# lzhangbj/deep_video_interpolation_extrapolation

Hardware: AMD Instinct MI355X
Metric: train frames/s (256x512 len-3 clips) (higher is better)
Workload: dtype bf16; 1 GPU; InterNet int_5_len_3 train step 256x512 bf16; per_gpu_batch=8, global_batch=8, parallelism=dp1, step=eager, executor side-stream lanes

## Files before the change

deep_video_interpolation_extrapolation_amd/_lib.py:

```python
import ctypes
import os
import threading

import torch

LIB_PATH = os.path.join(os.path.dirname(os.path.abspath(__file__)), "libdvie.so")

DVIE_OK = 0
DVIE_EINVAL = 1001
F32, BF16 = 0, 1
ACT_NONE, ACT_LRELU, ACT_ELU, ACT_RELU, ACT_TANH = 0, 1, 2, 3, 4
EW_FUSE, EW_UPT, EW_POOL, EW_POOLT, EW_COPY, EW_L1SIGN, EW_NCHW, EW_TONCHW, EW_MASK, EW_IM2COL, EW_LABELS = range(11)
LOSS_L1, LOSS_GDL, LOSS_SSIM, LOSS_MSE, LOSS_CE, LOSS_L1NHWC, LOSS_COSNHWC, LOSS_IOU, LOSS_ARGMAX_IOU = range(9)
OP_CONV, OP_WGRAD, OP_WREDUCE, OP_COLSUM, OP_EW, OP_LOSS, OP_PACK = 1, 2, 3, 4, 5, 6, 7
OP_BN_FWD, OP_BN_BWD, OP_HEAD_FWD, OP_HEAD_BWD, OP_ATTN, OP_HEAD3_BWD, OP_SEGENC_FWD = 8, 9, 10, 11, 12, 13, 14
OP_SEGENC_BWD = 15
OP_WREDUCE_MULTI = 16
OP_COSFEAT = 17
COSFEAT_MAX_TAPS = 8
YUV_420, YUV_444 = 420, 444
(ATTN_L2NORM, ATTN_L2NORM_BWD, ATTN_CORR, ATTN_GATHER, ATTN_GATHER_T, ATTN_SOFTMAX, ATTN_SOFTMAX_BWD, ATTN_WNORM,
 ATTN_WNORM_BWD, ATTN_POOL, ATTN_POOL_T) = range(11)

vp = ctypes.c_void_p
# ... 214 lines not shown

class AttnDesc(ctypes.Structure):
    _fields_ = [
        ("a", vp), ("b0", vp), ("b1", vp), ("y", vp), ("res", vp), ("z", vp),
        ("a_ld", i64), ("b_ld", i64), ("y_ld", i64), ("res_ld", i64), ("z_ld", i64),
        ("op", i32), ("n", i32), ("h", i32), ("w", i32),
        ("c", i32), ("wh", i32), ("ww", i32), ("nhalf", i32),
        ("half0", i32), ("act", i32), ("dact", i32), ("beta", i32),
        ("dtype", i32), ("pad0", i32),
        ("alpha", f32), ("pad1", f32),
    ]


class PackList(ctypes.Structure):
    _fields_ = [("descs_dev", vp), ("n", i32), ("blocks", i32)]


class Head3BwdDesc(ctypes.Structure):
    _fields_ = [
        ("g", vp), ("h", vp), ("wd", vp), ("dh", vp), ("ws", vp),
        ("g_ld", i64), ("h_ld", i64), ("dh_ld", i64),
        ("n", i32), ("hgt", i32), ("wid", i32), ("c", i32),
        ("cout", i32), ("kpad", i32), ("dy0", i32), ("dx0", i32),
        ("splits", i32), ("dact", i32),
        ("alpha", f32), ("pad0", f32),
    ]


class SegencDesc(ctypes.Structure):
    _fields_ = [
        ("inp", vp), ("e1", vp), ("e2", vp), ("out", vp), ("w0", vp), ("w2", vp), ("w4", vp),
        ("b0", vp), ("b2", vp), ("b4", vp),
        ("in_ld", i64), ("e1_ld", i64), ("e2_ld", i64), ("out_ld", i64),
        ("n", i32), ("h", i32), ("w", i32), ("kpad0", i32), ("kpad2", i32), ("kpad4", i32),
    ]


class SegencBwdDesc(ctypes.Structure):
    _fields_ = [
        ("dout", vp), ("e2", vp), ("e1", vp), ("inp", vp), ("w4d", vp), ("w2d", vp),
        ("dw4", vp), ("dw2", vp), ("dw0", vp), ("db4", vp), ("db2", vp), ("db0", vp),
        ("dout_ld", i64), ("e2_ld", i64), ("e1_ld", i64), ("in_ld", i64),
        ("n", i32), ("h", i32), ("w", i32), ("kpad4", i32), ("kpad2", i32), ("slabs", i32),
    ]


class WreduceMultiDesc(ctypes.Structure):
    _fields_ = [("descs", vp), ("n", i32), ("pad", i32)]


class _OpUnion(ctypes.Union):
    _fields_ = [
        ("conv", ConvDesc), ("wgrad", WgradDesc), ("wreduce", WreduceDesc), ("colsum", ColsumDesc),
        ("ew", EwDesc), ("loss", LossDesc), ("pack", PackList), ("bn", BnDesc), ("head", HeadDesc),
        ("attn", AttnDesc), ("head3", Head3BwdDesc), ("segenc", SegencDesc), ("segenc_bwd", SegencBwdDesc),
        ("wreduce_multi", WreduceMultiDesc), ("cosfeat", CosFeatDesc),
    ]


class Op(ctypes.Structure):
    _fields_ = [("kind", i32), ("lane", i32), ("u", _OpUnion)]


_ABI = {0: Op, OP_CONV: ConvDesc, OP_WGRAD: WgradDesc, OP_WREDUCE: WreduceDesc, OP_COLSUM: ColsumDesc,
        OP_EW: EwDesc, OP_LOSS: LossDesc, OP_PACK: PackDesc, OP_BN_FWD: BnDesc, OP_HEAD_FWD: HeadDesc,
        OP_ATTN: AttnDesc, OP_HEAD3_BWD: Head3BwdDesc, OP_SEGENC_FWD: SegencDesc, OP_SEGENC_BWD: SegencBwdDesc, OP_WREDUCE_MULTI: WreduceMultiDesc,
        OP_COSFEAT: CosFeatDesc, 100: WarpDesc, 101: SoftmaxDesc, 102: SnLayer, 103: ClipDesc,
        104: SynthLoadDesc, 105: SynthFinishDesc, 106: SynthBridgeDesc, 107: SynthScoreDesc,
        108: SynthLoadPadDesc, 109: SynthFinishCropDesc, 110: SynthVggLoadDesc}
_ABI_MORE = {111: SynthMsssimDesc, 112: SynthYuvDesc}

EXPORTS = [
    "dvie_conv2d_fwd", "dvie_conv2d_wgrad", "dvie_wgrad_splits_hint", "dvie_wgrad_slabs", "dvie_wgrad_reduce", "dvie_wgrad_reduce_multi", "dvie_colsum", "dvie_pack_weights",
    "dvie_ew", "dvie_loss", "dvie_loss_partial_count", "dvie_loss_ws_floats", "dvie_warp_fwd",
    "dvie_warp_bwd", "dvie_adamax", "dvie_scale", "dvie_run_ops", "dvie_abi_sizeof", "dvie_version",
    "dvie_last_error", "dvie_bn_fwd", "dvie_bn_bwd", "dvie_bn_partial_splits", "dvie_head_fwd", "dvie_head_bwd",
    "dvie_softmax_fwd", "dvie_softmax_bwd", "dvie_adam", "dvie_sn_fwd", "dvie_sn_bwd", "dvie_reparam_fwd",
    "dvie_reparam_bwd", "dvie_warp_ws_floats", "dvie_clip_prep", "dvie_attn", "dvie_step_inc", "dvie_adamax_dev",
    "dvie_adam_dev", "dvie_mfma_probe", "dvie_launch_probe", "dvie_sum_f32", "dvie_wgrad_bias_slabs", "dvie_head3_bwd",
    "dvie_segenc_fwd", "dvie_segenc_bwd", "dvie_pack_blocks", "dvie_trace_kernels", "dvie_traced_kernels",
    "dvie_synth_load", "dvie_synth_finish", "dvie_synth_bridge", "dvie_synth_score", "dvie_synth_score_ws_bytes",
    "dvie_synth_load_pad", "dvie_synth_finish_crop", "dvie_conv_zbits", "dvie_bn_partial_doubles",
    "dvie_synth_vgg_load", "dvie_cosfeat", "dvie_cosfeat_blocks", "dvie_synth_msssim", "dvie_synth_msssim_ws_bytes",
    "dvie_synth_yuv2rgb", "dvie_synth_rgb2yuv",
]

_lib = None
_lock = threading.Lock()


class DvieError(RuntimeError):
    pass


def load():
    global _lib
    if _lib is not None:
        return _lib
    with _lock:
        if _lib is not None:
            return _lib
        if not os.path.exists(LIB_PATH):
            raise DvieError(
                f"{LIB_PATH} is missing: build it with `python -c 'import __graft_entry__ as g; g.build()'` "
                "(there is no non-HIP fallback)")
        lib = ctypes.CDLL(LIB_PATH)
        lib.dvie_abi_sizeof.restype = ctypes.c_size_t
        lib.dvie_abi_sizeof.argtypes = [i32]
        for which, st in {**_ABI, **_ABI_MORE}.items():
            got = lib.dvie_abi_sizeof(which)
            if got != ctypes.sizeof(st):
                raise DvieError(f"ABI mismatch for {st.__name__}: C {got} vs ctypes {ctypes.sizeof(st)}")
        lib.dvie_version.restype = ctypes.c_char_p
        lib.dvie_last_error.restype = ctypes.c_char_p
        for name in ("dvie_conv2d_fwd", "dvie_conv2d_wgrad", "dvie_wgrad_reduce", "dvie_colsum", "dvie_ew",
                     "dvie_loss", "dvie_warp_fwd", "dvie_warp_bwd", "dvie_bn_fwd", "dvie_bn_bwd", "dvie_head_fwd",
                     "dvie_head_bwd", "dvie_softmax_fwd", "dvie_softmax_bwd", "dvie_clip_prep", "dvie_attn",
                     "dvie_head3_bwd", "dvie_segenc_fwd", "dvie_segenc_bwd", "dvie_synth_load", "dvie_synth_finish",
                     "dvie_synth_bridge", "dvie_synth_score", "dvie_synth_load_pad", "dvie_synth_finish_crop",
                     "dvie_synth_vgg_load", "dvie_cosfeat", "dvie_synth_msssim", "dvie_synth_yuv2rgb",
                     "dvie_synth_rgb2yuv"):
            getattr(lib, name).argtypes = [vp, vp]
            getattr(lib, name).restype = i32
        lib.dvie_pack_weights.argtypes = [vp, i32, i32, vp]
        lib.dvie_wgrad_reduce_multi.argtypes = [vp, i32, vp]
        lib.dvie_wgrad_reduce_multi.restype = i32
        lib.dvie_trace_kernels.argtypes = [i32]
        lib.dvie_trace_kernels.restype = i32
        lib.dvie_traced_kernels.argtypes = []
        lib.dvie_traced_kernels.restype = ctypes.c_char_p
        for name in ("dvie_wgrad_splits_hint", "dvie_wgrad_slabs", "dvie_bn_partial_splits", "dvie_pack_blocks",
                     "dvie_conv_zbits", "dvie_cosfeat_blocks"):
            getattr(lib, name).argtypes = [vp]
            getattr(lib, name).restype = i32
        lib.dvie_run_ops.argtypes = [vp, i32, vp]
        lib.dvie_loss_partial_count.argtypes = [vp]
        lib.dvie_loss_partial_count.restype = ctypes.c_size_t
        lib.dvie_warp_ws_floats.argtypes = [vp]
        lib.dvie_warp_ws_floats.restype = ctypes.c_size_t
        lib.dvie_loss_ws_floats.argtypes = [vp]
        lib.dvie_loss_ws_floats.restype = ctypes.c_size_t
        lib.dvie_bn_partial_doubles.argtypes = [vp]
        lib.dvie_bn_partial_doubles.restype = ctypes.c_size_t
        lib.dvie_synth_score_ws_bytes.argtypes = [vp]
        lib.dvie_synth_score_ws_bytes.restype = ctypes.c_size_t
        lib.dvie_synth_msssim_ws_bytes.argtypes = [vp]
        lib.dvie_synth_msssim_ws_bytes.restype = ctypes.c_size_t
        lib.dvie_adamax.argtypes = [vp, vp, vp, vp, i64, f32, f32, f32, f32, f32, vp]
        lib.dvie_scale.argtypes = [vp, i64, f32, vp]
        lib.dvie_adam.argtypes = [vp, vp, vp, vp, i64, f32, f32, f32, f32, f32, vp]
        f64 = ctypes.c_double
        lib.dvie_adamax_dev.argtypes = [vp, vp, vp, vp, i64, f64, f64, f64, f64, f64, vp, vp]
        lib.dvie_adam_dev.argtypes = [vp, vp, vp, vp, i64, f64, f64, f64, f64, f64, vp, vp]
        lib.dvie_step_inc.argtypes = [vp, vp]
        lib.dvie_mfma_probe.argtypes = [vp, i32, i32, vp]
        lib.dvie_mfma_probe.restype = i32
        lib.dvie_launch_probe.argtypes = [i32, i32, vp]
        lib.dvie_launch_probe.restype = i32
        lib.dvie_sum_f32.argtypes = [vp, i32, vp, vp]
        lib.dvie_sum_f32.restype = i32
        lib.dvie_wgrad_bias_slabs.argtypes = [vp]
        lib.dvie_wgrad_bias_slabs.restype = i32
        for name in ("dvie_sn_fwd", "dvie_sn_bwd"):
            getattr(lib, name).argtypes = [vp, i32, vp, vp]
            getattr(lib, name).restype = i32
        lib.dvie_reparam_fwd.argtypes = [vp, vp, vp, vp, i64, vp]
        lib.dvie_reparam_bwd.argtypes = [vp, vp, vp, vp, vp, i64, i32, vp]
        lib.dvie_reparam_fwd.restype = lib.dvie_reparam_bwd.restype = i32
        _lib = lib
        return lib


def check(rc, what=""):
    if rc != DVIE_OK:
        msg = load().dvie_last_error().decode(errors="replace") if rc == DVIE_EINVAL else f"hipError {rc}"
        raise DvieError(f"{what}: {msg}")


def stream_ptr(device=None):
    return torch.cuda.current_stream(device).cuda_stream


def require_gpu(t):
    if not t.is_cuda:
        raise DvieError("dvie ops run on the MI355X only: tensor is on %s (no CPU fallback)" % t.device)
```

deep_video_interpolation_extrapolation_amd/csrc/conv1x1.hip:

```cpp
#include <stdlib.h>

#include "conv_epilogue.h"

namespace dvie {

typedef __attribute__((address_space(3))) void* lds_ptr_1x1;

#define DVIE_VMCNT1(N) __builtin_amdgcn_s_waitcnt(((N) & 15) | (((N) >> 4) << 14) | (7 << 4) | (15 << 8))

__device__ __forceinline__ void transpose8x8(i32x4 (&ob)[8], int lane) {
  const int b = lane & 7;
#pragma unroll
  for (int d = 4; d >= 1; d >>= 1) {
    const bool up = (b & d) != 0;
#pragma unroll
    for (int k = 0; k < 8; ++k) {
      if (k & d) continue;
      i32x4 t, r;
#pragma unroll
      for (int e = 0; e < 4; ++e) t[e] = up ? ob[k][e] : ob[k + d][e];
#pragma unroll
      for (int e = 0; e < 4; ++e) r[e] = __shfl_xor(t[e], d);
#pragma unroll
      for (int e = 0; e < 4; ++e) {
// ... 750 lines not shown
      if (p.act == DVIE_ACT_LRELU) switch (dbg_env() & 7) {
#define DVIE_RING_AB(V)                                                                                                \
  case V:                                                                                                              \
    DVIE_LAUNCH((conv1x1_ring_kernel<TMC, NWP, MI, NWC, DVIE_ACT_LRELU, V>), dim3(256), dim3(64 * NW), 0, s, p, n_ct, \
                n_tiles);                                                                                              \
    return;
          DVIE_RING_AB(1) DVIE_RING_AB(2) DVIE_RING_AB(3) DVIE_RING_AB(4) DVIE_RING_AB(5) DVIE_RING_AB(6) DVIE_RING_AB(7)
#undef DVIE_RING_AB
          default: break;
        }
#endif
      if (p.act == DVIE_ACT_LRELU && p.zbits)
        DVIE_LAUNCH((conv1x1_ring_kernel<TMC, NWP, MI, NWC, DVIE_ACT_LRELU, 0, true>), dim3(256), dim3(64 * NW), 0, s, p, n_ct, n_tiles);
      else if (p.act == DVIE_ACT_LRELU)
        DVIE_LAUNCH((conv1x1_ring_kernel<TMC, NWP, MI, NWC, DVIE_ACT_LRELU>), dim3(256), dim3(64 * NW), 0, s, p, n_ct, n_tiles);
      else
        DVIE_LAUNCH((conv1x1_ring_kernel<TMC, NWP, MI, NWC, DVIE_ACT_NONE>), dim3(256), dim3(64 * NW), 0, s, p, n_ct, n_tiles);
      return;
    }
  }
  if constexpr (NS >= 2 && NS <= 5 && MI * TMC <= 4) {
    const int per_cu = 163840 / C::SMEM;
    const int G = 256 * (per_cu > 2 ? 2 : per_cu);
    if (p.c > KC && n_tiles > G) {
      DVIE_LAUNCH((conv1x1_persist_kernel<TMC, NS, KC, NWP, MI, NWC>), dim3(G), dim3(64 * NW), 0, s, p, n_ct,
                         n_tiles);
      return;
    }
  }
  const bool ident = ident_out(p);
  int pre = 0;
  if constexpr (NS == 1) {
    if (ident && p.c <= KC) {
      pre = MI * TMC > 4 ? 0 : (p.res ? 1 : 0) | (p.beta ? 2 : 0) | (p.dact ? 4 : 0);
      if ((pre & 4) && zb_reads(p)) pre |= 8;
      if (p.zbits && p.act) pre |= 16;
    }
  }
  if constexpr (NS == 1 && MI == 1 && 2 * TMC == 8) {
    if (ident && ce_env_on() && p.cout % C::BC == 0) {
      switch (pre) {
#define DVIE_CE_CASE(V)                                                                                              \
  case V:                                                                                                            \
    DVIE_LAUNCH((conv1x1_kernel<TMC, NS, KC, NWP, MI, NWC, false, PreOk<V, NS, MI * TMC, TMC>::v, true>), dim3(n_tiles), \
                       dim3(64 * NW), 0, s, p, n_ct, n_tiles, 0);                                                     \
    return;
        DVIE_CE_CASE(0) DVIE_CE_CASE(1) DVIE_CE_CASE(2) DVIE_CE_CASE(3) DVIE_CE_CASE(4)
        DVIE_CE_CASE(5) DVIE_CE_CASE(6) DVIE_CE_CASE(7)
        DVIE_CE_CASE(12) DVIE_CE_CASE(13) DVIE_CE_CASE(14) DVIE_CE_CASE(15) DVIE_CE_CASE(16) DVIE_CE_CASE(17)
#undef DVIE_CE_CASE
      }
    }
  }
  switch (pre) {
#define DVIE_PRE_CASE(V)                                                                                          \
  case V:                                                                                                        \
    DVIE_LAUNCH((conv1x1_kernel<TMC, NS, KC, NWP, MI, NWC, false, PreOk<V, NS, MI * TMC, TMC>::v>), dim3(n_tiles), \
                       dim3(64 * NW), 0, s, p, n_ct, n_tiles, dbg_env());                                                   \
    break;
    DVIE_PRE_CASE(1) DVIE_PRE_CASE(2) DVIE_PRE_CASE(3) DVIE_PRE_CASE(4) DVIE_PRE_CASE(5)
    DVIE_PRE_CASE(6) DVIE_PRE_CASE(7)
    DVIE_PRE_CASE(12) DVIE_PRE_CASE(13) DVIE_PRE_CASE(14) DVIE_PRE_CASE(15) DVIE_PRE_CASE(16) DVIE_PRE_CASE(17)
#undef DVIE_PRE_CASE
    default:
      DVIE_LAUNCH((conv1x1_kernel<TMC, NS, KC, NWP, MI, NWC, false>), dim3(n_tiles), dim3(64 * NW), 0, s, p, n_ct, n_tiles, dbg_env());
  }
}

static bool takes_1x1(const dvie_conv_desc& p) {
  if (p.dtype != DVIE_BF16 || p.th != 1 || p.tw != 1) return false;
  if (p.sy != 1 || p.sx != 1 || p.dy0 != 0 || p.dx0 != 0 || p.ih != p.oh || p.iw != p.ow) return false;
  if (p.osy < 1 || p.osx < 1 || p.ory < 0 || p.orx < 0) return false;
  if (p.c % 64 != 0 && p.c > 64) return false;
  if ((long long)p.n * p.oh * p.ow >= (1LL << 31)) return false;
  return true;
}

int conv1x1_zbits(const dvie_conv_desc& p) {
  if (!takes_1x1(p)) return -1;
  if (zb_writes(p)) return tile_1x1(p) == T_WIDE ? 2 : 1;
  return zb_reads(p);
}

bool conv1x1_launch(const dvie_conv_desc& p, hipStream_t s) {
  if (!takes_1x1(p)) return false;
  switch (tile_1x1(p)) {
    case T_2_1: launch_1x1<2, 1>(p, s); break;
    case T_2_3: launch_1x1<2, 3>(p, s); break;
    case T_4_3: launch_1x1<4, 3>(p, s); break;
    case T_4_1: launch_1x1<4, 1>(p, s); break;
    case T_WIDE: launch_1x1<4, 2, 64, 4, 2, 2>(p, s); break;
  }
  return true;
}

}
```

deep_video_interpolation_extrapolation_amd/csrc/warp_optim.hip:

```cpp
#include <stdlib.h>

#include <algorithm>

#include "common.h"

namespace dvie {

__device__ __forceinline__ float linspace_pm1(int i, int n) {
  if (n <= 1) return -1.f;
  const float step = 2.f / (float)(n - 1);
  return (i < n / 2) ? __builtin_fmaf(step, (float)i, -1.f) : __builtin_fmaf(-step, (float)(n - 1 - i), 1.f);
}

__device__ __forceinline__ float unnorm(float g, int size, int ac) {
  return ac ? ((g + 1.f) / 2.f) * (float)(size - 1) : ((g + 1.f) * (float)size - 1.f) / 2.f;
}

struct WarpTap {
  int x0, y0;
  float ix, iy, wnw, wne, wsw, wse;
  bool vx0, vx1, vy0, vy1;
};

__device__ __forceinline__ WarpTap warp_tap(int x, int y, float fx, float fy, int w, int h, int ac) {
  WarpTap t;
  const float gx = linspace_pm1(x, w) - fx;
  const float gy = linspace_pm1(y, h) - fy;
  t.ix = unnorm(gx, w, ac);
  t.iy = unnorm(gy, h, ac);
  t.x0 = (int)floorf(t.ix);
  t.y0 = (int)floorf(t.iy);
  const int x1 = t.x0 + 1, y1 = t.y0 + 1;
  t.wnw = ((float)x1 - t.ix) * ((float)y1 - t.iy);
  t.wne = (t.ix - (float)t.x0) * ((float)y1 - t.iy);
  t.wsw = ((float)x1 - t.ix) * (t.iy - (float)t.y0);
  t.wse = (t.ix - (float)t.x0) * (t.iy - (float)t.y0);
  t.vx0 = t.x0 >= 0 && t.x0 < w;
  t.vx1 = x1 >= 0 && x1 < w;
  t.vy0 = t.y0 >= 0 && t.y0 < h;
  t.vy1 = y1 >= 0 && y1 < h;
  return t;
}

__device__ __forceinline__ __amdgpu_buffer_rsrc_t warp_plane(const float* im, long long hw) {
  return __builtin_amdgcn_make_buffer_rsrc((void*)im, 0, (int)(hw * 4), 0x00020000);
}

__device__ __forceinline__ void warp_corners(__amdgpu_buffer_rsrc_t im, const WarpTap& t, int w, float& a, float& b,
                                             float& c, float& d, bool pair = false) {
  constexpr unsigned kOut = 0x80000000u;
  const unsigned r0 = (unsigned)(t.y0 * w), r1 = (unsigned)((t.y0 + 1) * w);
  if (pair) {
    const auto u = __builtin_amdgcn_raw_buffer_load_b64(im, t.vy0 ? (r0 + t.x0) * 4u : kOut, 0, 0);
    const auto v = __builtin_amdgcn_raw_buffer_load_b64(im, t.vy1 ? (r1 + t.x0) * 4u : kOut, 0, 0);
    a = __uint_as_float(u[0]);
    b = __uint_as_float(u[1]);
    c = __uint_as_float(v[0]);
    d = __uint_as_float(v[1]);
    return;
  }
  const unsigned oa = (t.vy0 && t.vx0) ? (r0 + t.x0) * 4u : kOut;
  const unsigned ob = (t.vy0 && t.vx1) ? (r0 + t.x0 + 1) * 4u : kOut;
  const unsigned oc = (t.vy1 && t.vx0) ? (r1 + t.x0) * 4u : kOut;
  const unsigned od = (t.vy1 && t.vx1) ? (r1 + t.x0 + 1) * 4u : kOut;
  a = __builtin_bit_cast(float, __builtin_amdgcn_raw_buffer_load_b32(im, oa, 0, 0));
  b = __builtin_bit_cast(float, __builtin_amdgcn_raw_buffer_load_b32(im, ob, 0, 0));
  c = __builtin_bit_cast(float, __builtin_amdgcn_raw_buffer_load_b32(im, oc, 0, 0));
  d = __builtin_bit_cast(float, __builtin_amdgcn_raw_buffer_load_b32(im, od, 0, 0));
}

__device__ __forceinline__ float warp_blend(float a, float b, float c, float d, const WarpTap& t) {
  float v = 0.f;
  v += a * t.wnw;
  v += b * t.wne;
  v += c * t.wsw;
  v += d * t.wse;
  return v;
}

template <int CC, int LAUX = 0, int SAUX = 0, int WPB = 4>
__global__ __launch_bounds__(64 * WPB) void warp_fwd_kernel(const dvie_warp_desc p, int xcd) {
  const int segs = (p.w + 255) >> 8;
  const long long hw = (long long)p.h * p.w;
  const int waves = p.n * p.h * segs;
  const int lane = threadIdx.x & 63;
// ... 415 lines not shown
  if (n == 0) return DVIE_OK;
  DVIE_LAUNCH(adamax_kernel, dim3(grid_for(n)), dim3(256), 0, (hipStream_t)stream, p, g, m, u, n, clr, b1, b2,
                     eps, wd, (const float*)nullptr, 0.0, 0.0);
  DVIE_RETURN_LAUNCH();
}

int dvie_adamax_dev(float* p, const float* g, float* m, float* u, long long n, double lr, double b1, double b2,
                    double eps, double wd, const float* step, void* stream) {
  DVIE_CHECK_ARG(p && g && m && u && step && n >= 0, "adamax_dev: args");
  if (n == 0) return DVIE_OK;
  DVIE_LAUNCH(adamax_kernel, dim3(grid_for(n)), dim3(256), 0, (hipStream_t)stream, p, g, m, u, n, 0.f,
                     (float)b1, (float)b2, (float)eps, (float)wd, step, lr, b1);
  DVIE_RETURN_LAUNCH();
}

int dvie_step_inc(float* step, void* stream) {
  DVIE_CHECK_ARG(step, "step_inc: null");
  DVIE_LAUNCH(step_inc_kernel, dim3(1), dim3(64), 0, (hipStream_t)stream, step);
  DVIE_RETURN_LAUNCH();
}

int dvie_scale(float* p, long long n, float s, void* stream) {
  DVIE_CHECK_ARG(p && n >= 0, "scale: args");
  if (n == 0) return DVIE_OK;
  DVIE_LAUNCH(scale_kernel, dim3(grid_for(n)), dim3(256), 0, (hipStream_t)stream, p, n, s);
  DVIE_RETURN_LAUNCH();
}

}

namespace {
struct DevLanes {
  hipStream_t side = nullptr;
  hipEvent_t join = nullptr, tail = nullptr;
  bool ok = false;
};
thread_local DevLanes dev_lanes[64];

DevLanes* lanes_of_device() {
  int dev = 0;
  if (hipGetDevice(&dev) != hipSuccess || dev < 0 || dev >= 64) return nullptr;
  DevLanes& d = dev_lanes[dev];
  if (!d.ok) {
    int least = 0, greatest = 0;
    if (hipDeviceGetStreamPriorityRange(&least, &greatest) != hipSuccess) least = 0;
    if (hipStreamCreateWithPriority(&d.side, hipStreamNonBlocking, least) != hipSuccess ||
        hipEventCreateWithFlags(&d.join, hipEventDisableTiming) != hipSuccess ||
        hipEventCreateWithFlags(&d.tail, hipEventDisableTiming) != hipSuccess)
      return nullptr;
    d.ok = true;
  }
  return &d;
}

bool lanes_on() {
  const char* e = getenv("DVIE_OP_LANES");
  return !(e && *e == '0');
}

struct LaneRun {
  DevLanes* d = nullptr;
  hipStream_t main = nullptr;
  bool tail_fresh = false;
  bool used = false;

  hipError_t enter_weight() {
    hipError_t e = hipSuccess;
    if (!tail_fresh) {
      e = hipEventRecord(d->tail, main);
      if (e == hipSuccess) e = hipStreamWaitEvent(d->side, d->tail, 0);
      tail_fresh = true;
    }
    used = true;
    return e;
  }
  hipError_t finish() {
    if (!used) return hipSuccess;
    hipError_t e = hipEventRecord(d->join, d->side);
    return e == hipSuccess ? hipStreamWaitEvent(main, d->join, 0) : e;
  }
};
}

extern "C" {

int dvie_run_ops(const dvie_op* ops, int n, void* stream) {
  LaneRun lr;
  lr.main = (hipStream_t)stream;
  hipStreamCaptureStatus cap = hipStreamCaptureStatusNone;
  const bool capturing = hipStreamIsCapturing(lr.main, &cap) == hipSuccess && cap != hipStreamCaptureStatusNone;
  const bool lanes = lanes_on() && !capturing;
  auto finish = [&](int rc) {
    if (lr.d) {
      const hipError_t e = lr.finish();
      if (rc == DVIE_OK && e != hipSuccess) {
        set_error("run_ops: lane join failed");
        return (int)e;
      }
    }
    return rc;
  };
  for (int i = 0; i < n; ++i) {
    int rc = DVIE_OK;
    const dvie_op& o = ops[i];
    if (o.lane < 0 || o.lane > 1) {
      set_error("run_ops: lane %d of op %d out of range", o.lane, i);
      return finish(DVIE_EINVAL);
    }
    hipStream_t st = lr.main;
    if (lanes && o.lane == 1) {
      if (!lr.d) lr.d = lanes_of_device();
      if (!lr.d) {
        set_error("run_ops: side stream unavailable");
        return finish(DVIE_EINVAL);
      }
      if (lr.enter_weight() != hipSuccess) {
        set_error("run_ops: weight-lane wait failed at op %d", i);
        return finish(DVIE_EINVAL);
      }
      st = lr.d->side;
    } else {
      lr.tail_fresh = false;
    }
    void* s = (void*)st;
#ifdef DVIE_TIMING_DBG
    static const long long skip_kinds = getenv("DVIE_SKIP_KINDS") ? atoll(getenv("DVIE_SKIP_KINDS")) : 0;
    if ((skip_kinds >> o.kind) & 1) continue;
#endif
    switch (o.kind) {
      case DVIE_OP_CONV: rc = dvie_conv2d_fwd(&o.u.conv, s); break;
      case DVIE_OP_WGRAD: rc = dvie_conv2d_wgrad(&o.u.wgrad, s); break;
      case DVIE_OP_WREDUCE: rc = dvie_wgrad_reduce(&o.u.wreduce, s); break;
      case DVIE_OP_WREDUCE_MULTI: rc = dvie_wgrad_reduce_multi(o.u.wreduce_multi.descs, o.u.wreduce_multi.n, s); break;
      case DVIE_OP_COLSUM: rc = dvie_colsum(&o.u.colsum, s); break;
      case DVIE_OP_EW: rc = dvie_ew(&o.u.ew, s); break;
      case DVIE_OP_LOSS: rc = dvie_loss(&o.u.loss, s); break;
      case DVIE_OP_PACK: rc = dvie_pack_weights(o.u.pack.descs_dev, o.u.pack.n, o.u.pack.blocks, s); break;
      case DVIE_OP_BN_FWD: rc = dvie_bn_fwd(&o.u.bn, s); break;
      case DVIE_OP_BN_BWD: rc = dvie_bn_bwd(&o.u.bn, s); break;
      case DVIE_OP_HEAD_FWD: rc = dvie_head_fwd(&o.u.head, s); break;
      case DVIE_OP_HEAD_BWD: rc = dvie_head_bwd(&o.u.head, s); break;
      case DVIE_OP_ATTN: rc = dvie_attn(&o.u.attn, s); break;
      case DVIE_OP_HEAD3_BWD: rc = dvie_head3_bwd(&o.u.head3, s); break;
      case DVIE_OP_SEGENC_FWD: rc = dvie_segenc_fwd(&o.u.segenc, s); break;
      case DVIE_OP_SEGENC_BWD: rc = dvie_segenc_bwd(&o.u.segenc_bwd, s); break;
      case DVIE_OP_COSFEAT: rc = dvie_cosfeat(&o.u.cosfeat, s); break;
      default: set_error("run_ops: unknown op kind %d at %d", o.kind, i); return finish(DVIE_EINVAL);
    }
    if (rc != DVIE_OK) {
      if (rc == DVIE_EINVAL) {
        char buf[512];
        snprintf(buf, sizeof(buf), "op %d (kind %d): %s", i, o.kind, dvie_last_error());
        set_error("%s", buf);
      }
      return finish(rc);
    }
  }
  return finish(DVIE_OK);
}

size_t dvie_abi_sizeof(int which) {
  switch (which) {
    case 0: return sizeof(dvie_op);
    case DVIE_OP_CONV: return sizeof(dvie_conv_desc);
    case DVIE_OP_WGRAD: return sizeof(dvie_wgrad_desc);
    case DVIE_OP_WREDUCE: return sizeof(dvie_wreduce_desc);
    case DVIE_OP_WREDUCE_MULTI: return sizeof(dvie_wreduce_multi_desc);
    case DVIE_OP_COLSUM: return sizeof(dvie_colsum_desc);
    case DVIE_OP_EW: return sizeof(dvie_ew_desc);
    case DVIE_OP_LOSS: return sizeof(dvie_loss_desc);
    case DVIE_OP_PACK: return sizeof(dvie_pack_desc);
    case DVIE_OP_BN_FWD: return sizeof(dvie_bn_desc);
    case DVIE_OP_HEAD_FWD: return sizeof(dvie_head_desc);
    case DVIE_OP_ATTN: return sizeof(dvie_attn_desc);
    case DVIE_OP_HEAD3_BWD: return sizeof(dvie_head3_bwd_desc);
    case DVIE_OP_SEGENC_FWD: return sizeof(dvie_segenc_desc);
    case DVIE_OP_SEGENC_BWD: return sizeof(dvie_segenc_bwd_desc);
    case DVIE_OP_COSFEAT: return sizeof(dvie_cosfeat_desc);
    case 100: return sizeof(dvie_warp_desc);
    case 101: return sizeof(dvie_softmax_desc);
    case 102: return sizeof(dvie_sn_layer);
    case 103: return sizeof(dvie_clip_desc);
    case 104: return sizeof(dvie_synth_load_desc);
    case 105: return sizeof(dvie_synth_finish_desc);
    case 106: return sizeof(dvie_synth_bridge_desc);
    case 107: return sizeof(dvie_synth_score_desc);
    case 108: return sizeof(dvie_synth_load_pad_desc);
    case 109: return sizeof(dvie_synth_finish_crop_desc);
    case 110: return sizeof(dvie_synth_vgg_load_desc);
    case 111: return sizeof(dvie_synth_msssim_desc);
    case 112: return sizeof(dvie_synth_yuv_desc);
    default: return 0;
  }
}

const char* dvie_version(void) { return "dvie 0.1.0 gfx950"; }

}
```

include/dvie.h:

```cpp
#ifndef DVIE_H
#define DVIE_H

#include <stddef.h>
#include <stdint.h>

#ifdef __cplusplus
extern "C" {
#endif

#define DVIE_OK 0
#define DVIE_EINVAL 1001

#define DVIE_F32 0
#define DVIE_BF16 1

#define DVIE_ACT_NONE 0
#define DVIE_ACT_LRELU 1
#define DVIE_ACT_ELU 2
#define DVIE_ACT_RELU 3
#define DVIE_ACT_TANH 4

typedef struct dvie_conv_desc {
  const void* x;
  const void* w;
  void* y;
  const float* bias;
  const void* res;
  const void* z;
  long long x_ld, y_ld, res_ld, z_ld;
  int n, ih, iw, c;
  int kpad, cout;
  int oh, ow, sy, sx;
  int th, tw, dy0, dx0, ddy, ddx;
  int yh, yw, osy, osx, ory, orx;
  int act, dact, beta, dtype;
  int out_f32;
  float alpha;
  int phc;
  int pad1;
  void* zbits;
  long long zbits_ld;
} dvie_conv_desc;

int dvie_conv2d_fwd(const dvie_conv_desc* d, void* stream);

int dvie_conv_zbits(const dvie_conv_desc* d);

typedef struct dvie_wgrad_desc {
  const void* g;
  const void* x;
  float* ws;
  long long g_ld, x_ld;
  int n, oh, ow, cout;
  int ih, iw, c, sy;
  int sx, th, tw, dy0;
  int dx0, ddy, ddx, splits;
  int dtype;
  int tmap;
  float* bws;
  int ws_taps;
  int pad1;
} dvie_wgrad_desc;

int dvie_conv2d_wgrad(const dvie_wgrad_desc* d, void* stream);

int dvie_wgrad_bias_slabs(const dvie_wgrad_desc* d);

int dvie_wgrad_splits_hint(const dvie_wgrad_desc* d);

int dvie_wgrad_slabs(const dvie_wgrad_desc* d);

typedef struct dvie_wreduce_desc {
  const float* ws;
  float* dw;
  const int* cmap;
  int splits, ws_rows, ws_k, co_off;
  int cout_p, cin_p, kh_n, kw_n;
  int c, beta;
} dvie_wreduce_desc;

int dvie_wgrad_reduce(const dvie_wreduce_desc* d, void* stream);

int dvie_wgrad_reduce_multi(const dvie_wreduce_desc* descs, int n, void* stream);
typedef struct dvie_wreduce_multi_desc {
  const dvie_wreduce_desc* descs;
  int n, pad;
} dvie_wreduce_multi_desc;

typedef struct dvie_colsum_desc {
  const void* g;
  float* ws;
  long long g_ld;
  long long rows;
  int c, splits, dtype, pad0;
} dvie_colsum_desc;

int dvie_colsum(const dvie_colsum_desc* d, void* stream);

typedef struct dvie_pack_desc {
  const float* src;
  void* dst;
  const int* cmap;
  int rows, kpad, c, mode;
  int th, tw, kh0, kw0;
  int dkh, dkw, cout_s, cin_s;
  int kh_s, kw_s, dtype, blk0;
} dvie_pack_desc;

int dvie_pack_weights(const dvie_pack_desc* descs_dev, int n, int blocks, void* stream);

int dvie_pack_blocks(const dvie_pack_desc* d);

#define DVIE_EW_FUSE 0
#define DVIE_EW_UPT 1
#define DVIE_EW_POOL 2
#define DVIE_EW_POOLT 3
#define DVIE_EW_COPY 4
#define DVIE_EW_L1SIGN 5
#define DVIE_EW_NCHW 6
#define DVIE_EW_TONCHW 7
#define DVIE_EW_MASK 8
#define DVIE_EW_IM2COL 9
#define DVIE_EW_LABELS 10

typedef struct dvie_ew_desc {
  void* y;
  const void* src0;
  const void* src1;
  const void* src2;
  const void* res;
// ... 338 lines not shown
  uint8_t* label;
  uint8_t* label_canvas;
  int n, h, w, hp, wp;
  int rgb_ld, seg_ld, n_classes;
  int pad0;
} dvie_synth_finish_crop_desc;

int dvie_synth_load_pad(const dvie_synth_load_pad_desc* d, void* stream);
int dvie_synth_finish_crop(const dvie_synth_finish_crop_desc* d, void* stream);

typedef struct dvie_synth_bridge_desc {
  const float* rgb;
  const float* seg;
  void* dst;
  long long npix;
  int rgb_ld, seg_ld, dst_ld, dtype;
  int n_rgb, rgb_w, seg_w, pad0;
} dvie_synth_bridge_desc;

int dvie_synth_bridge(const dvie_synth_bridge_desc* d, void* stream);

typedef struct dvie_synth_score_desc {
  const uint8_t* pred;
  const uint8_t* gt;
  const uint8_t* pred_label;
  const uint8_t* gt_label;
  long long* sse;
  double* ssim;
  long long* agree;
  long long* valid;
  long long* inter;
  long long* uni;
  void* ws;
  long long pred_s0, pred_s1, gt_s0, gt_s1;
  long long pred_label_s0, pred_label_s1, gt_label_s0, gt_label_s1;
  int n0, n1, h, w, n_classes, pad0;
} dvie_synth_score_desc;

size_t dvie_synth_score_ws_bytes(const dvie_synth_score_desc* d);
int dvie_synth_score(const dvie_synth_score_desc* d, void* stream);

typedef struct dvie_synth_vgg_load_desc {
  const uint8_t* pred;
  const uint8_t* gt;
  void* out;
  const void* lut;
  long long pred_s0, pred_s1, gt_s0, gt_s1;
  int n0, n1, h, w, h16, w16, dtype;
  int img0, n_out, pad0;
} dvie_synth_vgg_load_desc;

int dvie_synth_vgg_load(const dvie_synth_vgg_load_desc* d, void* stream);

typedef struct dvie_synth_msssim_desc {
  const uint8_t* pred;
  const uint8_t* gt;
  double* msssim;
  double* parts;
  void* ws;
  long long pred_s0, pred_s1, gt_s0, gt_s1;
  int n0, n1, h, w, scales, pad0;
} dvie_synth_msssim_desc;

size_t dvie_synth_msssim_ws_bytes(const dvie_synth_msssim_desc* d);
int dvie_synth_msssim(const dvie_synth_msssim_desc* d, void* stream);

#define DVIE_YUV_420 420
#define DVIE_YUV_444 444

typedef struct dvie_synth_yuv_desc {
  uint8_t* yuv;
  uint8_t* rgb;
  long long yuv_stride;
  long long rgb_stride, rgb_row_stride;
  int n, h, w, layout, yo, pad0;
  int table[12];
} dvie_synth_yuv_desc;

int dvie_synth_yuv2rgb(const dvie_synth_yuv_desc* d, void* stream);
int dvie_synth_rgb2yuv(const dvie_synth_yuv_desc* d, void* stream);

int dvie_run_ops(const dvie_op* ops, int n, void* stream);

size_t dvie_abi_sizeof(int which);
const char* dvie_version(void);
const char* dvie_last_error(void);

int dvie_trace_kernels(int on);
const char* dvie_traced_kernels(void);

#ifdef __cplusplus
}
#endif

#endif
```

Before: 257.7 frames/s.

## Fuse back-to-back 1x1 convs (c<=64 -> 256 -> 64) into one chained kernel

Adds a fused HIP kernel that runs two consecutive bf16 1x1 convolutions in one launch. The 256-channel intermediate tile stays in LDS for the second GEMM, but the first conv's output is still written to global memory. The op runner detects chainable conv pairs, skipping over side-lane weight ops only when their memory does not overlap the second conv's output. The aim is to remove one kernel launch and the global re-read of the intermediate, at the cost of a large LDS footprint per block and strict eligibility checks.

```diff
diff --git a/deep_video_interpolation_extrapolation_amd/_lib.py b/deep_video_interpolation_extrapolation_amd/_lib.py
--- a/deep_video_interpolation_extrapolation_amd/_lib.py
+++ b/deep_video_interpolation_extrapolation_amd/_lib.py
@@ -320,7 +320,7 @@
     "dvie_synth_load", "dvie_synth_finish", "dvie_synth_bridge", "dvie_synth_score", "dvie_synth_score_ws_bytes",
     "dvie_synth_load_pad", "dvie_synth_finish_crop", "dvie_conv_zbits", "dvie_bn_partial_doubles",
     "dvie_synth_vgg_load", "dvie_cosfeat", "dvie_cosfeat_blocks", "dvie_synth_msssim", "dvie_synth_msssim_ws_bytes",
-    "dvie_synth_yuv2rgb", "dvie_synth_rgb2yuv",
+    "dvie_synth_yuv2rgb", "dvie_synth_rgb2yuv", "dvie_conv_chain", "dvie_conv2d_chain", "dvie_ops_chain_pairs",
 ]
 
 _lib = None
@@ -372,6 +372,12 @@
             getattr(lib, name).argtypes = [vp]
             getattr(lib, name).restype = i32
         lib.dvie_run_ops.argtypes = [vp, i32, vp]
+        lib.dvie_conv_chain.argtypes = [vp, vp]
+        lib.dvie_conv_chain.restype = i32
+        lib.dvie_conv2d_chain.argtypes = [vp, vp, vp]
+        lib.dvie_conv2d_chain.restype = i32
+        lib.dvie_ops_chain_pairs.argtypes = [vp, i32, vp]
+        lib.dvie_ops_chain_pairs.restype = i32
         lib.dvie_loss_partial_count.argtypes = [vp]
         lib.dvie_loss_partial_count.restype = ctypes.c_size_t
         lib.dvie_warp_ws_floats.argtypes = [vp]
diff --git a/deep_video_interpolation_extrapolation_amd/csrc/conv1x1.hip b/deep_video_interpolation_extrapolation_amd/csrc/conv1x1.hip
--- a/deep_video_interpolation_extrapolation_amd/csrc/conv1x1.hip
+++ b/deep_video_interpolation_extrapolation_amd/csrc/conv1x1.hip
@@ -856,6 +856,19 @@
   return zb_reads(p);
 }
 
+int conv1x1_route(const dvie_conv_desc& p, int* zb) {
+  *zb = 0;
+  if (!takes_1x1(p)) return -1;
+  *zb = (zb_reads(p) ? 1 : 0) | (zb_writes(p) ? 2 : 0);
+  switch (tile_1x1(p)) {
+    case T_2_1: return 21;
+    case T_2_3: return 23;
+    case T_4_3: return 43;
+    case T_4_1: return 41;
+    default: return 42;
+  }
+}
+
 bool conv1x1_launch(const dvie_conv_desc& p, hipStream_t s) {
   if (!takes_1x1(p)) return false;
   switch (tile_1x1(p)) {
diff --git a/deep_video_interpolation_extrapolation_amd/csrc/conv_chain.hip b/deep_video_interpolation_extrapolation_amd/csrc/conv_chain.hip
--- /dev/null
+++ b/deep_video_interpolation_extrapolation_amd/csrc/conv_chain.hip
@@ -0,0 +1,348 @@
+#include "conv_epilogue.h"
+
+namespace dvie {
+
+int conv1x1_route(const dvie_conv_desc& p, int* zb);
+
+#define DVIE_CHAIN_VMCNT(N) __builtin_amdgcn_s_waitcnt(((N) & 15) | (((N) >> 4) << 14) | (7 << 4) | (15 << 8))
+
+struct ChainCfg {
+  static constexpr int BP = 64;
+  static constexpr int XSZ = BP * 128;
+  static constexpr int W1SZ = 256 * 128;
+  static constexpr int W2SZ = 64 * 512;
+  static constexpr int MSZ = BP * 512;
+  static constexpr int X0 = 0, W1 = 2 * XSZ, W2 = W1 + W1SZ, M0 = W2 + W2SZ;
+  static constexpr int SMEM = M0 + 2 * MSZ;
+  static constexpr int GRID = 256;
+};
+
+template <int AM, bool RES, bool BZ>
+__global__ __launch_bounds__(512) void conv1x1_chain_kernel(const dvie_conv_desc a_in, const dvie_conv_desc b_in, int n_tiles) {
+  typedef ChainCfg C;
+  dvie_conv_desc a = a_in, b = b_in;
+  a.act = a_in.act == DVIE_ACT_LRELU ? DVIE_ACT_LRELU : a_in.act == DVIE_ACT_RELU ? DVIE_ACT_RELU : DVIE_ACT_NONE;
+  b.act = b_in.act == DVIE_ACT_LRELU ? DVIE_ACT_LRELU : b_in.act == DVIE_ACT_RELU ? DVIE_ACT_RELU : DVIE_ACT_NONE;
+  a.dact = a_in.dact == DVIE_ACT_LRELU ? DVIE_ACT_LRELU : a_in.dact == DVIE_ACT_RELU ? DVIE_ACT_RELU : DVIE_ACT_NONE;
+  b.dact = b_in.dact == DVIE_ACT_LRELU ? DVIE_ACT_LRELU : b_in.dact == DVIE_ACT_RELU ? DVIE_ACT_RELU : DVIE_ACT_NONE;
+  __shared__ __attribute__((aligned(1024))) char smem[C::SMEM];
+  const int tid = threadIdx.x, lane = tid & 63;
+  const int wave = __builtin_amdgcn_readfirstlane(tid >> 6);
+  const int r32 = lane & 31, hh = lane >> 5;
+  const unsigned OOB = 0xFFFFFFF0u;
+
+  const int G = gridDim.x;
+  const int g8 = blockIdx.x & 7, i8 = blockIdx.x >> 3;
+  const int q8 = G >> 3, r8 = G & 7;
+  const int bid = (g8 < r8 ? g8 * (q8 + 1) : r8 * (q8 + 1) + (g8 - r8) * q8) + i8;
+  const int npix = a.n * a.oh * a.ow;
+  const int my_tiles = bid < n_tiles ? (n_tiles - 1 - bid) / G + 1 : 0;
+  if (my_tiles == 0) return;
+
+  const unsigned long long np1 = (unsigned long long)npix - 1;
+  auto rsrc = [](const void* ptr, unsigned long long bytes) {
+    return __builtin_amdgcn_make_buffer_rsrc((void*)ptr, 0, ptr ? (int)bytes : 0, 0x00020000);
+  };
+  const __amdgpu_buffer_rsrc_t rx = rsrc(a.x, np1 * a.x_ld * 2ull + a.c * 2ull);
+  const __amdgpu_buffer_rsrc_t rw1 = rsrc(a.w, 256ull * a.kpad * 2ull);
+  const __amdgpu_buffer_rsrc_t rw2 = rsrc(b.w, 64ull * b.kpad * 2ull);
+  const __amdgpu_buffer_rsrc_t rres = rsrc(RES ? a.res : nullptr, np1 * a.res_ld * 2ull + 512ull);
+  const __amdgpu_buffer_rsrc_t ry = rsrc(a.y, np1 * a.y_ld * 2ull + 512ull);
+  const __amdgpu_buffer_rsrc_t rzb = rsrc((AM == 1 || AM == 2) ? a.zbits : nullptr, np1 * a.zbits_ld + 32ull);
+  const __amdgpu_buffer_rsrc_t rza = rsrc(AM == 3 ? a.z : nullptr, np1 * a.z_ld * 2ull + 512ull);
+  const __amdgpu_buffer_rsrc_t ry2 = rsrc(b.y, np1 * b.y_ld * 2ull + 128ull);
+  const __amdgpu_buffer_rsrc_t rz2 = rsrc(BZ ? b.z : nullptr, np1 * b.z_ld * 2ull + 128ull);
+
+  const int xrow = wave * 8 + (lane >> 3);
+  const int xcs = (lane & 7) ^ ((xrow >> 1) & 7);
+  const bool xc_ok = xcs * 8 < a.c;
+  int mrow[4], mcs[4];
+#pragma unroll
+  for (int q = 0; q < 4; ++q) {
+    mrow[q] = (wave + 8 * q) * 2 + (lane >> 5);
+    mcs[q] = (lane & 31) ^ (mrow[q] & 15);
+  }
+  auto issue_tile = [&](int i) {
+    const int p0 = (bid + i * G) * C::BP;
+    const int buf = i & 1;
+    lds_dma16(rx, smem + C::X0 + buf * C::XSZ + wave * 1024,
+              (xc_ok && p0 + xrow < npix) ? (unsigned)(p0 + xrow) * (unsigned)a.x_ld * 2u + xcs * 16u : OOB);
+    if constexpr (RES) {
+#pragma unroll
+      for (int q = 0; q < 4; ++q)
+        lds_dma16(rres, smem + C::M0 + buf * C::MSZ + (wave + 8 * q) * 1024,
+                  p0 + mrow[q] < npix ? (unsigned)(p0 + mrow[q]) * (unsigned)a.res_ld * 2u + mcs[q] * 16u : OOB);
+    }
+  };
+
+  const int wp = wave & 1, wc = wave >> 1;
+  const int prow = 32 * wp + r32;
+  const int psw = prow & 15;
+  int xf[4], wf[4];
+#pragma unroll
+  for (int s = 0; s < 4; ++s) {
+    xf[s] = prow * 128 + (((2 * s + hh) ^ ((prow >> 1) & 7)) << 4);
+    wf[s] = (64 * wc + r32) * 128 + (((2 * s + hh) ^ ((r32 >> 1) & 7)) << 4);
+  }
+  const int w2row = 32 * (wave >> 1) + r32;
+
+  struct Pre {
+    i32x2 zb;
+    i32x4 za[4], z2[2];
+  };
+  auto load_pre = [&](int i, Pre& o) {
+    const int p0 = (bid + i * G) * C::BP;
+    const int pix = p0 + prow;
+    const bool ok = pix < npix;
+    if constexpr (AM == 2)
+      o.zb = __builtin_bit_cast(i32x2, __builtin_amdgcn_raw_buffer_load_b64(
+                                           rzb, ok ? (unsigned)pix * (unsigned)a.zbits_ld + 8u * wc : OOB, 0, 0));
+    if constexpr (AM == 3) {
+#pragma unroll
+      for (int k = 0; k < 4; ++k) {
+        const int co = 64 * wc + 16 * k + 8 * hh;
+        o.za[k] = __builtin_bit_cast(i32x4, __builtin_amdgcn_raw_buffer_load_b128(
+                                                rza, ok ? ((unsigned)pix * (unsigned)a.z_ld + co) * 2u : OOB, 0, 0));
+      }
+    }
+    if constexpr (BZ) {
+      if (wave < 4) {
+#pragma unroll
+        for (int P = 0; P < 2; ++P) {
+          const int co = 32 * (wave >> 1) + 16 * P + 8 * hh;
+          o.z2[P] = __builtin_bit_cast(i32x4, __builtin_amdgcn_raw_buffer_load_b128(
+                                                  rz2, ok ? ((unsigned)pix * (unsigned)b.z_ld + co) * 2u : OOB, 0, 0));
+        }
+      }
+    }
+  };
+
+#pragma unroll
+  for (int q = 0; q < 4; ++q) {
+    const int row = (wave + 8 * q) * 8 + (lane >> 3);
+    const int cs = (lane & 7) ^ ((row >> 1) & 7);
+    lds_dma16(rw1, smem + C::W1 + (wave + 8 * q) * 1024, cs * 8 < a.c ? (unsigned)row * (unsigned)a.kpad * 2u + cs * 16u : OOB);
+  }
+#pragma unroll
+  for (int q = 0; q < 4; ++q)
+    lds_dma16(rw2, smem + C::W2 + (wave + 8 * q) * 1024, (unsigned)mrow[q] * (unsigned)b.kpad * 2u + mcs[q] * 16u);
+  issue_tile(0);
+  Pre pre = {}, nxt = {};
+  load_pre(0, pre);
+  float bias_a[4][8], bias_b[2][8];
+#pragma unroll
+  for (int k = 0; k < 4; ++k)
+#pragma unroll
+    for (int e = 0; e < 8; ++e) bias_a[k][e] = 0.f;
+#pragma unroll
+  for (int P = 0; P < 2; ++P)
+#pragma unroll
+    for (int e = 0; e < 8; ++e) bias_b[P][e] = 0.f;
+  if (a.bias) {
+#pragma unroll
+    for (int k = 0; k < 4; ++k) add_f32x8(bias_a[k], a.bias + 64 * wc + 16 * k + 8 * hh);
+  }
+  if (b.bias && wave < 4) {
+#pragma unroll
+    for (int P = 0; P < 2; ++P) add_f32x8(bias_b[P], b.bias + 32 * (wave >> 1) + 16 * P + 8 * hh);
+  }
+
+  __builtin_amdgcn_s_waitcnt(0);
+  for (int i = 0; i < my_tiles; ++i) {
+    const int buf = i & 1;
+    const int p0 = (bid + i * G) * C::BP;
+    if (i > 0) {
+      if (wave < 4)
+        DVIE_CHAIN_VMCNT(4 + (AM == 1 ? 1 : 0) + 2);
+      else
+        DVIE_CHAIN_VMCNT(4 + (AM == 1 ? 1 : 0));
+    }
+    __builtin_amdgcn_s_barrier();
+    if (i + 1 < my_tiles) {
+      issue_tile(i + 1);
+      load_pre(i + 1, nxt);
+    }
+
+    const char* X = smem + C::X0 + buf * C::XSZ;
+    const char* W1 = smem + C::W1;
+    char* M = smem + C::M0 + buf * C::MSZ;
+    f32x16 acc[2];
+#pragma unroll
+    for (int j = 0; j < 2; ++j)
+#pragma unroll
+      for (int e = 0; e < 16; ++e) acc[j][e] = 0.f;
+#pragma unroll
+    for (int s = 0; s < 4; ++s) {
+      const i32x4 bq = *(const i32x4*)(X + xf[s]);
+      i32x4 aq[2];
+#pragma unroll
+      for (int j = 0; j < 2; ++j) aq[j] = *(const i32x4*)(W1 + wf[s] + j * 32 * 128);
+#pragma unroll
+      for (int j = 0; j < 2; ++j)
+        acc[j] = __builtin_amdgcn_mfma_f32_32x32x16_bf16(__builtin_bit_cast(bf16x8, aq[j]), __builtin_bit_cast(bf16x8, bq),
+                                                         acc[j], 0, 0, 0);
+    }
+
+    {
+      const int pix = p0 + prow;
+      const bool ok = pix < npix;
+      unsigned zq = 0;
+#pragma unroll
+      for (int j = 0; j < 2; ++j) {
+        float v[2][8];
+        acc_rows8(acc[j], v);
+#pragma unroll
+        for (int P = 0; P < 2; ++P) {
+          const int co = 64 * wc + 32 * j + 16 * P + 8 * hh;
+          char* m = M + prow * 512 + (((co >> 3) ^ psw) << 4);
+          float* w = v[P];
+          if (a.bias) {
+#pragma unroll
+            for (int e = 0; e < 8; ++e) w[e] += bias_a[2 * j + P][e];
+          }
+          i32x4 o;
+          if constexpr (AM == 2) {
+            const i32x4 r = RES ? *(const i32x4*)m : i32x4{0, 0, 0, 0};
+            o = epi8_regs_bits<RES, false>(w, a, &r, nullptr, ((unsigned)pre.zb[j] >> (8 * (2 * P + hh))) & 0xffu);
+          } else {
+            const i32x4 r = RES ? *(const i32x4*)m : i32x4{0, 0, 0, 0};
+            o = epi8_regs<RES, false, AM == 3>(w, a, &r, nullptr, &pre.za[2 * j + P]);
+          }
+          *(i32x4*)m = o;
+          if constexpr (AM == 1) zq |= sign_bits8(o) << (8 * (2 * j + P));
+          __builtin_amdgcn_raw_buffer_store_b128(o, ry, ok ? ((unsigned)pix * (unsigned)a.y_ld + co) * 2u : OOB, 0, 0);
+        }
+      }
+      if constexpr (AM == 1) {
+        const unsigned other = (unsigned)__shfl_xor((int)zq, 32);
+        const unsigned ev = hh ? other : zq, od = hh ? zq : other;
+        const unsigned e2 = ev >> (16 * hh), o2 = od >> (16 * hh);
+        const unsigned z0 = (e2 & 0xffu) | ((o2 & 0xffu) << 8) | ((e2 & 0xff00u) << 8) | ((o2 & 0xff00u) << 16);
+        __builtin_amdgcn_raw_buffer_store_b32(z0, rzb, ok ? (unsigned)pix * (unsigned)a.zbits_ld + 8u * wc + 4u * hh : OOB, 0, 0);
+      }
+    }
+    __builtin_amdgcn_s_waitcnt(0xC07F);
+    __builtin_amdgcn_s_barrier();
+
+    if (wave < 4) {
+      const char* W2 = smem + C::W2;
+      f32x16 acc2;
+#pragma unroll
+      for (int e = 0; e < 16; ++e) acc2[e] = 0.f;
+      const char* mb = M + prow * 512;
+      const char* wb = W2 + w2row * 512;
+      const int wsw = w2row & 15;
+#pragma unroll
+      for (int s = 0; s < 16; ++s) {
+        const i32x4 bq = *(const i32x4*)(mb + (((2 * s + hh) ^ psw) << 4));
+        const i32x4 aq = *(const i32x4*)(wb + (((2 * s + hh) ^ wsw) << 4));
+        acc2 = __builtin_amdgcn_mfma_f32_32x32x16_bf16(__builtin_bit_cast(bf16x8, aq), __builtin_bit_cast(bf16x8, bq), acc2,
+                                                       0, 0, 0);
+      }
+      float v[2][8];
+      acc_rows8(acc2, v);
+      const int pix = p0 + prow;
+      const bool ok = pix < npix;
+#pragma unroll
+      for (int P = 0; P < 2; ++P) {
+        const int co = 32 * (wave >> 1) + 16 * P + 8 * hh;
+        float* w = v[P];
+        if (b.bias) {
+#pragma unroll
+          for (int e = 0; e < 8; ++e) w[e] += bias_b[P][e];
+        }
+        const i32x4 o = epi8_regs<false, false, BZ>(w, b, nullptr, nullptr, &pre.z2[P]);
+        __builtin_amdgcn_raw_buffer_store_b128(o, ry2, ok ? ((unsigned)pix * (unsigned)b.y_ld + co) * 2u : OOB, 0, 0);
+      }
+    }
+    pre = nxt;
+  }
+  __builtin_amdgcn_s_waitcnt(0);
+}
+
+static bool sign_or_none(int v) { return v == DVIE_ACT_NONE || v == DVIE_ACT_LRELU || v == DVIE_ACT_RELU; }
+
+static bool overlaps(const void* p, unsigned long long pb, const void* q, unsigned long long qb) {
+  if (!p || !q || !pb || !qb) return false;
+  const uintptr_t a0 = (uintptr_t)p, b0 = (uintptr_t)q;
+  return a0 < b0 + qb && b0 < a0 + pb;
+}
+
+struct Span {
+  const void* p;
+  unsigned long long bytes;
+};
+
+static int chain_variant(const dvie_conv_desc& a, const dvie_conv_desc& b) {
+  int za = 0, zb = 0;
+  if (conv1x1_route(a, &za) != 41 || conv1x1_route(b, &zb) != 23) return 0;
+  auto plain = [](const dvie_conv_desc& p) {
+    return p.x && p.w && p.y && !p.out_f32 && !p.beta && !p.phc && p.osy == 1 && p.osx == 1 && p.ory == 0 && p.orx == 0 &&
+           p.yh == p.oh && p.yw == p.ow && p.n > 0 && p.oh > 0 && p.ow > 0 && p.c > 0 && p.c % 8 == 0 &&
+           p.kpad % 64 == 0 && p.kpad >= p.c && p.x_ld % 8 == 0 && p.x_ld >= p.c && p.y_ld % 8 == 0 && p.y_ld >= p.cout &&
+           ((uintptr_t)p.x & 15) == 0 && ((uintptr_t)p.w & 15) == 0 && ((uintptr_t)p.y & 15) == 0 &&
+           ((uintptr_t)p.bias & 15) == 0 && sign_or_none(p.act) && sign_or_none(p.dact) && !(p.act && p.dact);
+  };
+  if (!plain(a) || !plain(b)) return 0;
+  if (a.n != b.n || a.oh != b.oh || a.ow != b.ow) return 0;
+  if (b.x != a.y || b.x_ld != a.y_ld || a.cout != 256 || b.c != 256 || a.c > 64 || b.cout != 64) return 0;
+  if (b.res || dvie_conv_zbits(&b) != 0) return 0;
+  const bool a_bits_r = a.dact && (za & 1), a_bits_w = a.act && (za & 2);
+  if (a.res && (a.res_ld % 8 != 0 || a.res_ld < 256 || ((uintptr_t)a.res & 15))) return 0;
+  if (a.dact && !a_bits_r && (!a.z || a.z_ld % 8 != 0 || a.z_ld < 256 || ((uintptr_t)a.z & 15))) return 0;
+  if (b.dact && (!b.z || b.z_ld % 8 != 0 || b.z_ld < 64 || ((uintptr_t)b.z & 15))) return 0;
+  if ((a_bits_r || a_bits_w) && a.zbits_ld < 32) return 0;
+
+  const unsigned long long np1 = (unsigned long long)a.n * a.oh * a.ow - 1;
+  const Span ax{a.x, np1 * a.x_ld * 2ull + a.c * 2ull}, aw{a.w, 256ull * a.kpad * 2ull}, ab{a.bias, 256ull * 4ull};
+  const Span ar{a.res, np1 * a.res_ld * 2ull + 512ull};
+  const Span az{(a.dact && !a_bits_r) ? a.z : nullptr, np1 * a.z_ld * 2ull + 512ull};
+  const Span azb{(a_bits_r || a_bits_w) ? a.zbits : nullptr, np1 * a.zbits_ld + 32ull};
+  const Span ay{a.y, np1 * a.y_ld * 2ull + 512ull};
+  const Span bw{b.w, 64ull * b.kpad * 2ull}, bb{b.bias, 64ull * 4ull};
+  const Span bz{b.dact ? b.z : nullptr, np1 * b.z_ld * 2ull + 128ull};
+  const Span by{b.y, np1 * b.y_ld * 2ull + 128ull};
+  for (const Span& s : {ax, aw, ar, az, azb, ay, bw, bz, by})
+    if (s.p && s.bytes >= 0xFFFFFF00ull) return 0;
+  for (const Span& o : {ay, a_bits_w ? azb : Span{nullptr, 0}})
+    for (const Span& s : {bw, bb, bz, by})
+      if (overlaps(o.p, o.bytes, s.p, s.bytes)) return 0;
+  for (const Span& s : {ax, aw, ab, ar, az, azb})
+    if (overlaps(by.p, by.bytes, s.p, s.bytes)) return 0;
+
+  const int am = a.dact ? (a_bits_r ? 2 : 3) : (a_bits_w ? 1 : 0);
+  return 1 + (am | (a.res ? 4 : 0) | (b.dact ? 8 : 0));
+}
+
+}
+
+using namespace dvie;
+
+extern "C" int dvie_conv_chain(const dvie_conv_desc* a, const dvie_conv_desc* b) {
+  return a && b && chain_variant(*a, *b) != 0;
+}
+
+extern "C" int dvie_conv2d_chain(const dvie_conv_desc* a, const dvie_conv_desc* b, void* stream) {
+  DVIE_CHECK_ARG(a && b, "conv chain: null descriptor");
+  const int v = chain_variant(*a, *b);
+  DVIE_CHECK_ARG(v != 0, "conv chain: not a chainable pair (dvie_conv_chain): bf16 1x1 c<=64 -> 256 -> 64 on the "
+                         "same pixels, b.x = a.y, beta 0, bf16 outputs, disjoint operands");
+  hipStream_t s = (hipStream_t)stream;
+  dvie_conv_desc pa = *a;
+  if (!((v - 1) & 3)) pa.zbits = nullptr;
+  const int npix = a->n * a->oh * a->ow;
+  const int n_tiles = (npix + ChainCfg::BP - 1) / ChainCfg::BP;
+  const int G = n_tiles < ChainCfg::GRID ? n_tiles : ChainCfg::GRID;
+  switch (v - 1) {
+#define DVIE_CHAIN_CASE(V)                                                                                          \
+  case V:                                                                                                           \
+    DVIE_LAUNCH((conv1x1_chain_kernel<(V) & 3, ((V) & 4) != 0, ((V) & 8) != 0>), dim3(G), dim3(512), 0, s, pa, *b, \
+                n_tiles);                                                                                           \
+    break;
+    DVIE_CHAIN_CASE(0) DVIE_CHAIN_CASE(1) DVIE_CHAIN_CASE(2) DVIE_CHAIN_CASE(3) DVIE_CHAIN_CASE(4) DVIE_CHAIN_CASE(5)
+    DVIE_CHAIN_CASE(6) DVIE_CHAIN_CASE(7) DVIE_CHAIN_CASE(8) DVIE_CHAIN_CASE(9) DVIE_CHAIN_CASE(10) DVIE_CHAIN_CASE(11)
+    DVIE_CHAIN_CASE(12) DVIE_CHAIN_CASE(13) DVIE_CHAIN_CASE(14) DVIE_CHAIN_CASE(15)
+#undef DVIE_CHAIN_CASE
+  }
+  DVIE_RETURN_LAUNCH();
+}
diff --git a/deep_video_interpolation_extrapolation_amd/csrc/warp_optim.hip b/deep_video_interpolation_extrapolation_amd/csrc/warp_optim.hip
--- a/deep_video_interpolation_extrapolation_amd/csrc/warp_optim.hip
+++ b/deep_video_interpolation_extrapolation_amd/csrc/warp_optim.hip
@@ -1,6 +1,7 @@
 #include <stdlib.h>
 
 #include <algorithm>
+#include <vector>
 
 #include "common.h"
 
@@ -582,11 +583,84 @@
 };
 }
 
+static bool chain_on() {
+  const char* e = getenv("DVIE_CHAIN");
+  return !(e && *e == '0');
+}
+
+struct OpSpan {
+  const void* p;
+  unsigned long long bytes;
+};
+static bool weight_op_spans(const dvie_op& o, std::vector<OpSpan>& v) {
+  auto reduce = [&](const dvie_wreduce_desc& d) {
+    v.push_back({d.ws, (unsigned long long)d.splits * d.ws_rows * d.ws_k * 4ull});
+    v.push_back({d.dw, (unsigned long long)d.cout_p * d.cin_p * d.kh_n * d.kw_n * 4ull});
+  };
+  switch (o.kind) {
+    case DVIE_OP_WGRAD: {
+      const dvie_wgrad_desc& d = o.u.wgrad;
+      const unsigned long long es = d.dtype == DVIE_BF16 ? 2 : 4;
+      const unsigned long long row = (unsigned long long)(d.ws_taps > 0 ? d.ws_taps : d.th * d.tw) * d.c;
+      v.push_back({d.g, ((unsigned long long)d.n * d.oh * d.ow - 1) * d.g_ld * es + d.cout * es});
+      v.push_back({d.x, ((unsigned long long)d.n * d.ih * d.iw - 1) * d.x_ld * es + d.c * es});
+      v.push_back({d.ws, (unsigned long long)dvie_wgrad_slabs(&d) * d.cout * row * 4ull});
+      if (d.bws) v.push_back({d.bws, (unsigned long long)dvie_wgrad_bias_slabs(&d) * d.cout * 4ull});
+      return true;
+    }
+    case DVIE_OP_WREDUCE: reduce(o.u.wreduce); return true;
+    case DVIE_OP_WREDUCE_MULTI:
+      for (int k = 0; k < o.u.wreduce_multi.n; ++k) reduce(o.u.wreduce_multi.descs[k]);
+      return true;
+    case DVIE_OP_COLSUM: {
+      const dvie_colsum_desc& d = o.u.colsum;
+      const unsigned long long es = d.dtype == DVIE_BF16 ? 2 : 4;
+      v.push_back({d.g, (unsigned long long)(d.rows - 1) * d.g_ld * es + d.c * es});
+      v.push_back({d.ws, (unsigned long long)d.splits * d.c * 4ull});
+      return true;
+    }
+    default: return false;
+  }
+}
+
 extern "C" {
+
+int dvie_ops_chain_pairs(const dvie_op* ops, int n, int* partner) {
+  int pairs = 0;
+  for (int i = 0; i < n; ++i) partner[i] = -1;
+  if (!chain_on()) return 0;
+  std::vector<OpSpan> sp;
+  for (int i = 0; i + 1 < n; ++i) {
+    if (partner[i] >= 0 || ops[i].kind != DVIE_OP_CONV || ops[i].lane != 0) continue;
+    int j = i + 1;
+    while (j < n && ops[j].lane == 1) ++j;
+    if (j >= n || ops[j].kind != DVIE_OP_CONV || ops[j].lane != 0) continue;
+    const dvie_conv_desc& a = ops[i].u.conv;
+    const dvie_conv_desc& b = ops[j].u.conv;
+    if (!dvie_conv_chain(&a, &b)) continue;
+    const uintptr_t y0 = (uintptr_t)b.y;
+    const unsigned long long yb = ((unsigned long long)b.n * b.yh * b.yw - 1) * b.y_ld * 2ull + b.cout * 2ull;
+    bool ok = true;
+    sp.clear();
+    for (int k = i + 1; k < j && ok; ++k) ok = weight_op_spans(ops[k], sp);
+    for (size_t k = 0; k < sp.size() && ok; ++k)
+      if (sp[k].p && sp[k].bytes && (uintptr_t)sp[k].p < y0 + yb && y0 < (uintptr_t)sp[k].p + sp[k].bytes) ok = false;
+    if (!ok) continue;
+    partner[i] = j;
+    partner[j] = i;
+    ++pairs;
+  }
+  return pairs;
+}
 
 int dvie_run_ops(const dvie_op* ops, int n, void* stream) {
   LaneRun lr;
   lr.main = (hipStream_t)stream;
+  std::vector<int> partner;
+  if (n > 1 && chain_on()) {
+    partner.resize(n);
+    if (dvie_ops_chain_pairs(ops, n, partner.data()) == 0) partner.clear();
+  }
   hipStreamCaptureStatus cap = hipStreamCaptureStatusNone;
   const bool capturing = hipStreamIsCapturing(lr.main, &cap) == hipSuccess && cap != hipStreamCaptureStatusNone;
   const bool lanes = lanes_on() && !capturing;
@@ -627,6 +701,10 @@
     static const long long skip_kinds = getenv("DVIE_SKIP_KINDS") ? atoll(getenv("DVIE_SKIP_KINDS")) : 0;
     if ((skip_kinds >> o.kind) & 1) continue;
 #endif
+    if (!partner.empty() && partner[i] >= 0) {
+      if (partner[i] < i) continue;
+      rc = dvie_conv2d_chain(&o.u.conv, &ops[partner[i]].u.conv, s);
+    } else
     switch (o.kind) {
       case DVIE_OP_CONV: rc = dvie_conv2d_fwd(&o.u.conv, s); break;
       case DVIE_OP_WGRAD: rc = dvie_conv2d_wgrad(&o.u.wgrad, s); break;
diff --git a/include/dvie.h b/include/dvie.h
--- a/include/dvie.h
+++ b/include/dvie.h
@@ -46,6 +46,9 @@
 
 int dvie_conv_zbits(const dvie_conv_desc* d);
 
+int dvie_conv_chain(const dvie_conv_desc* a, const dvie_conv_desc* b);
+int dvie_conv2d_chain(const dvie_conv_desc* a, const dvie_conv_desc* b, void* stream);
+
 typedef struct dvie_wgrad_desc {
   const void* g;
   const void* x;
@@ -550,6 +553,8 @@
 
 int dvie_run_ops(const dvie_op* ops, int n, void* stream);
 
+int dvie_ops_chain_pairs(const dvie_op* ops, int n, int* partner);
+
 size_t dvie_abi_sizeof(int which);
 const char* dvie_version(void);
 const char* dvie_last_error(void);
```

Measured after the change: 262.2 frames/s (median of 6 runs). +1.7%, better.
